# Siverteh/semantic-slam-master

Measured on AMD Instinct MI355X. Metric: frames/sec extract+match on TUM 640x480; match-index bit-exact vs CPU ref, higher is better.
Workload: dtype f32

## Files before the change

### include/sslam_hip.h

```cpp
#ifndef SSLAM_HIP_H
#define SSLAM_HIP_H

#include <stdint.h>

#ifdef __cplusplus
extern "C" {
#endif

#define SSLAM_OK 0
#define SSLAM_E_INVALID (-1)
#define SSLAM_E_UNSUPPORTED (-2)
#define SSLAM_E_LAUNCH (-3)

#define SSLAM_C 384
#define SSLAM_HID 384
#define SSLAM_D 128

int sslam_version(void);
const char *sslam_arch(void);
long long sslam_launch_count(void);

long long sslam_workspace_bytes(int n_frames, int G, int K, int n_pairs);
long long sslam_selector_saliency_workspace_bytes(int n_frames, int G);
long long sslam_sim_argmax_workspace_bytes(int n2, int n_pairs);

int sslam_test_set_knob(const char *name, long long value, int unset);

int sslam_pack_conv3x3_host(const float *w_host, int hs, float *out_host);
int sslam_pack_linear_host(const float *w_host, int n_out, int k_in, float *out_host);

#define SSLAM_MAX_TAPS 32
int sslam_resample_table_host(int in_size, int out_size, int filter, int32_t *bounds_host, int32_t *coefs_host,
                              int coefs_capacity);
int sslam_preprocess_u8(const uint8_t *img, int n, int h, int w, int size, const int32_t *bounds_h,
                        const int32_t *coefs_h, int ksize_h, const int32_t *bounds_v, const int32_t *coefs_v,
                        int ksize_v, float *out_chw, void *stream);
int sslam_preprocess_u8_patches(const uint8_t *img, int n, int h, int w, int size, const int32_t *bounds_h,
                                const int32_t *coefs_h, int ksize_h, const int32_t *bounds_v, const int32_t *coefs_v,
                                int ksize_v, void *out_patches_bf16, void *stream);

int sslam_bn_tokens(const float *tokens, int n_frames, int tokens_per_frame, int n_prefix, int group,
                    const float *gamma, const float *beta, const float *run_mean, const float *run_var, int train,
                    float eps, float *out_feat, float *out_mean, float *out_var, void *stream);

int sslam_selector_saliency(const float *feat, int n_frames, int G, const float *w1_packed, const float *b1,
                            const float *w2, const float *b2, int hs, float *sal, void *stream);
int sslam_selector_saliency_ws(const float *feat, int n_frames, int G, const float *w1_packed, const float *b1,
                               const float *w2, const float *b2, int hs, float *sal, void *workspace,
                               long long workspace_bytes, void *stream);

int sslam_f32_to_bf16(const float *in, void *out_bf16, long long n, void *stream);
int sslam_bn_tokens_bf16copy(const float *tokens, int n_frames, int tokens_per_frame, int n_prefix, int group,
                             const float *gamma, const float *beta, const float *run_mean, const float *run_var, int train,
                             float eps, float *out_feat, void *out_feat_bf16, float *out_mean, float *out_var, void *stream);
int sslam_pack_conv3x3_bf16_host(const float *w_host, int hs, void *out_bf16_host);
int sslam_selector_saliency_bf16(const void *feat_bf16, int n_frames, int G, const void *w1_packed_bf16, const float *b1,
                                 const float *w2, const float *b2, int hs, float *sal, void *stream);

int sslam_select_keypoints(const float *sal, int n_frames, int G, int K, int nms_radius, double min_score_percentile,
                           float *kp_xy, float *scores, int32_t *idx, float *kp_pixel, int32_t *status,
                           void *stream);

int sslam_gather(const float *feat, int n_frames, int G, const float *kp_xy, int K, float *out, void *stream);

typedef struct {
    int n_blocks;
    long long total;
    long long in_w, in_b;
    long long blk[8][8];
    long long out_w, out_b;
} sslam_refiner_layout_t;
int sslam_refiner_layout(int n_blocks, sslam_refiner_layout_t *layout_host);
int sslam_refiner_pack_host(const float *const *w_host, int n_blocks, float *out_host);
int sslam_refine(const float *x, long long rows, const float *packed, int n_blocks, float *desc, void *stream);

int sslam_gather_refine(const float *feat, int n_frames, int G, const float *kp_xy, int K, const float *packed,
                        int n_blocks, float *desc, void *stream);

long long sslam_refiner_bf16_bytes(int n_blocks);
int sslam_refiner_pack_bf16_host(const float *const *w_host, int n_blocks, void *out_host);
int sslam_refine_bf16(const float *x, long long rows, const void *packed_bf16, int n_blocks, float *desc, void *stream);
int sslam_gather_refine_bf16(const float *feat, int n_frames, int G, const float *kp_xy, int K, const void *packed_bf16,
                             int n_blocks, float *desc, void *stream);

int sslam_keypoint_intensity(const uint8_t *img, int n, int h, int w, int size, const int32_t *bounds_h,
                             const int32_t *coefs_h, int ksize_h, const int32_t *bounds_v, const int32_t *coefs_v,
                             int ksize_v, const float *kp_pixel, int K, float *out, void *stream);

int sslam_sim_argmax(const float *desc1, long long stride1, int n1, const float *desc2, long long stride2, int n2,
                     int n_pairs, int32_t *nn12, float *s12, int32_t *nn21, float *s21, float *second12, void *stream);
int sslam_sim_argmax_ws(const float *desc1, long long stride1, int n1, const float *desc2, long long stride2, int n2,
                        int n_pairs, int32_t *nn12, float *s12, int32_t *nn21, float *s21, float *second12,
                        void *workspace, long long workspace_bytes, void *stream);

int sslam_match_finalize(const int32_t *nn12, const float *s12, const int32_t *nn21, int n1, int n2, int n_pairs,
                         const float *scores1, long long sstride1, const float *scores2, long long sstride2,
                         const float *intensity1, const float *intensity2, float w_desc, float w_sal,
                         float min_saliency, float min_sim, float min_intensity, int64_t *matches, float *quality,
                         int32_t *count, void *stream);

typedef struct {
    const float *ln1_g, *ln1_b;
    const void *wqkv;
    const float *bqkv;
    const void *wo;
    const float *bo, *ln2_g, *ln2_b;
    const void *wup;
    const float *bup;
    const void *wdown;
    const float *bdown;
// ... 49 lines not shown
```

### semantic-slam-master_amd/csrc/common.h

```cpp
#pragma once

#include <hip/hip_runtime.h>
#include <stdint.h>

#include "../../include/sslam_hip.h"

typedef float f32x16 __attribute__((ext_vector_type(16)));
typedef float f32x4 __attribute__((ext_vector_type(4)));

extern long long g_sslam_launches;
static inline void sslam_count_launches(long long n) { __atomic_fetch_add(&g_sslam_launches, n, __ATOMIC_RELAXED); }

enum sslam_knob_id {
    KNOB_M1_VARIANT,
    KNOB_CONV_VARIANT,
    KNOB_CONV_LATENCY_ROWS,
    KNOB_CONV_LAT2_ROWS,
    KNOB_CONV_NO_HALO,
    KNOB_CONV_TAIL,
    KNOB_CONVBF_NO_HALO,
    KNOB_CONVBF_TAIL,
    KNOB_CONVBF_VARIANT,
    KNOB_VIT_NO_FUSED_MLP,
    KNOB_BN_FORM,
    KNOB_VIT_F32_NO_KEY_SPLIT,
    KNOB_RT_STOP,
    KNOB_COUNT
};
#define SSLAM_KNOB_UNSET (-0x7fffffffffffffffLL - 1)
extern long long g_sslam_knob[KNOB_COUNT];
static inline long long sslam_knob(int id, long long dflt) { const long long v = g_sslam_knob[id]; return v == SSLAM_KNOB_UNSET ? dflt : v; }
static inline bool sslam_knob_set(int id) { return g_sslam_knob[id] != SSLAM_KNOB_UNSET; }

#define SSLAM_CHECK_LAUNCH()                                   \
    do {                                                       \
        sslam_count_launches(1);                               \
        if (hipGetLastError() != hipSuccess) return SSLAM_E_LAUNCH; \
    } while (0)

__host__ __device__ inline int kp8(int k) { return (k & ~7) | ((k & 1) << 2) | ((k & 7) >> 1); }

__device__ __forceinline__ f32x16 mfma32(float a, float b, f32x16 c) {
    return __builtin_amdgcn_mfma_f32_32x32x2f32(a, b, c, 0, 0, 0);
}

__device__ __forceinline__ int crow(int r, int h) { return (r & 3) + 8 * (r >> 2) + 4 * h; }

__device__ __forceinline__ float bfly32(float v) {
    v = v + __shfl_xor(v, 16);
    v = v + __shfl_xor(v, 8);
    v = v + __shfl_xor(v, 4);
    v = v + __shfl_xor(v, 2);
    v = v + __shfl_xor(v, 1);
    return v;
}
__device__ __forceinline__ float bfly64(float v) {
    v = v + __shfl_xor(v, 32);
    return bfly32(v);
}
// ... 24 lines not shown
```

### semantic-slam-master_amd/csrc/lib.hip

```cpp
#include <stdlib.h>
#include <string.h>

#include "common.h"

long long g_sslam_launches = 0;
long long g_sslam_knob[KNOB_COUNT];

namespace {
long long g_knob_at_load[KNOB_COUNT];
const char *const kKnobNames[KNOB_COUNT] = {
    "SSLAM_M1_VARIANT",   "SSLAM_CONV_VARIANT",  "SSLAM_CONV_LATENCY_ROWS", "SSLAM_CONV_LAT2_ROWS",   "SSLAM_CONV_NO_HALO",
    "SSLAM_CONV_TAIL",    "SSLAM_CONVBF_NO_HALO", "SSLAM_CONVBF_TAIL",      "SSLAM_CONVBF_VARIANT",   "SSLAM_VIT_NO_FUSED_MLP",
    "SSLAM_BN_FORM",      "SSLAM_VIT_F32_NO_KEY_SPLIT", "SSLAM_RT_STOP"};
struct KnobInit {
    KnobInit() {
        for (int i = 0; i < KNOB_COUNT; i++) {
            const char *e = getenv(kKnobNames[i]);
            g_sslam_knob[i] = g_knob_at_load[i] = e ? atoll(e) : SSLAM_KNOB_UNSET;
        }
    }
} g_knob_init;
}

extern "C" int sslam_version(void) { return 300; }
extern "C" const char *sslam_arch(void) { return "gfx950"; }
extern "C" long long sslam_launch_count(void) { return __atomic_load_n(&g_sslam_launches, __ATOMIC_RELAXED); }

extern "C" long long sslam_workspace_bytes(int n_frames, int G, int K, int n_pairs) {
    if (n_frames <= 0 || G <= 0 || K <= 0 || n_pairs < 0) return SSLAM_E_INVALID;
    const long long a = sslam_selector_saliency_workspace_bytes(n_frames, G);
    const long long b = n_pairs > 0 ? sslam_sim_argmax_workspace_bytes(K, n_pairs) : 0;
    const long long m = a > b ? a : b;
    return (m + 255) & ~255LL;
}

extern "C" int sslam_test_set_knob(const char *name, long long value, int unset) {
    if (!name) return SSLAM_E_INVALID;
    for (int i = 0; i < KNOB_COUNT; i++)
        if (!strcmp(name, kKnobNames[i])) {
            g_sslam_knob[i] = unset ? g_knob_at_load[i] : value;
            return SSLAM_OK;
        }
    return SSLAM_E_INVALID;
}
```

### semantic-slam-master_amd/csrc/refine.hip

```cpp
#include "common.h"
#include "gather_taps.h"

namespace {

#ifndef SSLAM_REFINE_WMR
#define SSLAM_REFINE_WMR 1
#endif
constexpr int WMR = SSLAM_REFINE_WMR;
constexpr int RM = 32 * WMR;
constexpr int NTHR = 256 * WMR;
constexpr int HID = SSLAM_HID;
constexpr int LDH = HID + 4;
constexpr int NKG = HID / 8;
constexpr int H_FLOATS = RM * LDH;
constexpr int SCRATCH_FLOATS = 256;
constexpr int SMEM_FLOATS = H_FLOATS + SCRATCH_FLOATS;

struct RefArgs {
    const float *packed;
    sslam_refiner_layout_t lay;
};

typedef unsigned u32x4 __attribute__((ext_vector_type(4)));

// ... 28 lines not shown
    f32x4 an = *reinterpret_cast<const f32x4 *>(A);
#pragma unroll 1
    for (int g = 0; g < NKG; g += 3) {
        LOAD_B(b2, g + 2);
        __builtin_amdgcn_sched_barrier(0);
        STEP(b0, g);
        __builtin_amdgcn_sched_barrier(0);
        LOAD_B(b0, min(g + 3, NKG - 1));
        __builtin_amdgcn_sched_barrier(0);
        STEP(b1, g + 1);
        __builtin_amdgcn_sched_barrier(0);
        LOAD_B(b1, min(g + 4, NKG - 1));
        __builtin_amdgcn_sched_barrier(0);
        STEP(b2, g + 2);
        __builtin_amdgcn_sched_barrier(0);
    }
#undef LOAD_B
#undef STEP
}

template <int V>
struct IC {
    static constexpr int value = V;
};
template <int DW>
__device__ __forceinline__ void store_quad(unsigned row_lds, float y0, float y1, float y2, float y3) {
    asm volatile("ds_write2_b32 %0, %1, %2 offset0:%3 offset1:%4" ::"v"(row_lds), "v"(y0), "v"(y1), "n"(DW), "n"(DW + 4) : "memory");
    asm volatile("ds_write2_b32 %0, %1, %2 offset0:%3 offset1:%4" ::"v"(row_lds), "v"(y2), "v"(y3), "n"(DW + 1), "n"(DW + 5) : "memory");
}
__device__ __forceinline__ void lds_quads_done() { asm volatile("s_waitcnt lgkmcnt(0)" ::: "memory"); }
__device__ __forceinline__ unsigned lds_addr(const float *p) {
    return (unsigned)(size_t)(__attribute__((address_space(3))) const float *)p;
}
template <int I>
__device__ __forceinline__ void store_rows_from(unsigned row_lds, const f32x16 (&v)[3]) {
    if constexpr (I < 12) {
        constexpr int t = I / 4, q = I % 4;
        store_quad<32 * t + 8 * q>(row_lds, v[t][4 * q], v[t][4 * q + 1], v[t][4 * q + 2], v[t][4 * q + 3]);
        store_rows_from<I + 1>(row_lds, v);
    }
}
__device__ __forceinline__ void store_rows(float *H, int tid, const f32x16 (&v)[3]) {
    const int lane = tid & 63, wave = tid >> 6, r = lane & 31, h = lane >> 5, wn = wave & 3;
    store_rows_from<0>(lds_addr(H + r * LDH + wn * 96 + 2 * h), v);
    lds_quads_done();
}

__device__ __forceinline__ float row_total(float p, float *part, int tid) {
    const int lane = tid & 63, wave = tid >> 6, r = lane & 31, h = lane >> 5, wn = wave & 3;
    p = p + __shfl_xor(p, 32);
    if (h == 0) part[wn * 32 + r] = p;
    __syncthreads();
    return ((part[r] + part[32 + r]) + part[64 + r]) + part[96 + r];
}

__device__ __forceinline__ void layernorm_store(float *H, float *part0, float *part1, const float *__restrict__ gam,
                                                const float *__restrict__ bet, int tid, const f32x16 (&v)[3]) {
    const int lane = tid & 63, wave = tid >> 6, r = lane & 31, h = lane >> 5, wn = wave & 3;
    const float *gp = gam + wn * 96 + 4 * h, *bp = bet + wn * 96 + 4 * h;
    constexpr int AHEAD = 3;
    f32x4 g4[AHEAD], b4[AHEAD];
#define LN_REQ(i_)                                                                                       \
    {                                                                                                    \
        g4[(i_) % AHEAD] = *reinterpret_cast<const f32x4 *>(gp + 32 * ((i_) / 4) + 8 * ((i_) % 4));      \
        b4[(i_) % AHEAD] = *reinterpret_cast<const f32x4 *>(bp + 32 * ((i_) / 4) + 8 * ((i_) % 4));      \
    }
// ... 20 lines not shown
        constexpr int i = decltype(ic)::value, t = i / 4, qd = i % 4;
        const f32x4 gq = g4[i % AHEAD], bq = b4[i % AHEAD];
        float y[4];
#pragma unroll
        for (int j = 0; j < 4; j++) y[j] = __builtin_fmaf((v[t][4 * qd + j] - mean) * rstd, gq[j], bq[j]);
        if constexpr (i + AHEAD < 12) LN_REQ(i + AHEAD)
        __builtin_amdgcn_sched_barrier(0);
        store_quad<32 * t + 8 * qd>(row_lds, y[0], y[1], y[2], y[3]);
    };
    quad(IC<0>{}); quad(IC<1>{}); quad(IC<2>{}); quad(IC<3>{}); quad(IC<4>{}); quad(IC<5>{});
    quad(IC<6>{}); quad(IC<7>{}); quad(IC<8>{}); quad(IC<9>{}); quad(IC<10>{}); quad(IC<11>{});
    lds_quads_done();
#undef LN_REQ
}

#ifdef SSLAM_CLOCK_PROBE
__device__ unsigned long long g_probe_refine[8 * 4096];
#define PROBE_BEGIN() const unsigned long long pr_t0 = clock64(); unsigned long long pr_q = 0, pr_acc[6] = {0, 0, 0, 0, 0, 0}
#define PROBE(slot, stmt) { pr_q = clock64(); stmt; pr_acc[slot] += clock64() - pr_q; }
#define PROBE_END()                                                                                         \
    if (threadIdx.x == 0 && blockIdx.x < 4096) {                                                            \
        g_probe_refine[8 * blockIdx.x] = clock64() - pr_t0;                                                 \
        for (int i_ = 0; i_ < 6; i_++) g_probe_refine[8 * blockIdx.x + 1 + i_] = pr_acc[i_];                \
    }
#else
#define PROBE_BEGIN()
#define PROBE(slot, stmt) { stmt; }
#define PROBE_END()
#endif
#define PRIO_OTHER() __builtin_amdgcn_s_setprio(1)
#define PRIO_GEMM() __builtin_amdgcn_s_setprio(0)
enum { PR_GATHER = 0, PR_GEMM = 1, PR_LN = 2, PR_STORE = 3, PR_BARRIER = 4 };

__global__ __launch_bounds__(NTHR, WMR == 1 ? 3 : 2) void gather_refine_kernel(const float *__restrict__ feat, int G,
                                                             const float *__restrict__ kp_xy, int K,
                                                             const float *__restrict__ x_in, long long rows,
                                                             RefArgs args, float *__restrict__ desc) {
    __shared__ __attribute__((aligned(16))) float smem[SMEM_FLOATS];
    float *H = smem, *scratch = smem + H_FLOATS;
    const int tid = threadIdx.x;
    PROBE_BEGIN();
    PRIO_OTHER();
    long long R0;
    {
        const int n_tiles = gridDim.x, b = blockIdx.x, q = n_tiles / 8, rem = n_tiles % 8, x = b % 8;
        R0 = (long long)((x < rem ? x * (q + 1) : rem * (q + 1) + (x - rem) * q) + b / 8) * RM;
    }
    const float *pk = args.packed;
    const sslam_refiner_layout_t &L = args.lay;
    const __amdgpu_buffer_rsrc_t wrs = __builtin_amdgcn_make_buffer_rsrc(const_cast<float *>(pk), 0, (int)(L.total * 4), 0x00020000);

    {
        const int row = tid >> 3, part = tid & 7;
        long long R = R0 + row;
        if (R > rows - 1) R = rows - 1;
        float *dst = H + row * LDH;
        if (feat) {
            const long long f = R / K;
            const Taps t = make_taps(feat + f * G * G * SSLAM_C, G, kp_xy[2 * R], kp_xy[2 * R + 1]);
#pragma unroll
            for (int j = 0; j < 6; j++) {
                const int c0 = 8 * (j * 8 + part);
                float4 ev, od;
                kp8_split(blend4(t, c0), blend4(t, c0 + 4), ev, od);
                *reinterpret_cast<float4 *>(dst + c0) = ev;
                *reinterpret_cast<float4 *>(dst + c0 + 4) = od;
            }
        } else {
            const float *src = x_in + R * SSLAM_C;
#pragma unroll
            for (int j = 0; j < 6; j++) {
                const int c0 = 8 * (j * 8 + part);
                float4 ev, od;
                kp8_split(*reinterpret_cast<const float4 *>(src + c0), *reinterpret_cast<const float4 *>(src + c0 + 4), ev, od);
                *reinterpret_cast<float4 *>(dst + c0) = ev;
                *reinterpret_cast<float4 *>(dst + c0 + 4) = od;
            }
        }
    }
#ifdef SSLAM_CLOCK_PROBE
    pr_acc[PR_GATHER] = clock64() - pr_t0;
#endif
    PROBE(PR_BARRIER, __syncthreads();)

    float *part0 = scratch, *part1 = scratch + 128;
    f32x16 X[3], acc[3];
    PRIO_GEMM(); PROBE(PR_GEMM, gemm_lds<3>(H, wrs, (int)L.in_w * 4, pk + L.in_b, tid, acc);) PRIO_OTHER();
#pragma unroll
    for (int t = 0; t < 3; t++)
#pragma unroll
        for (int e = 0; e < 16; e++) X[t][e] = acc[t][e] > 0.0f ? acc[t][e] : 0.0f;

    for (int b = 0; b < L.n_blocks; b++) {
        PROBE(PR_LN, layernorm_store(H, part0, part1, pk + L.blk[b][0], pk + L.blk[b][1], tid, X);)
        PROBE(PR_BARRIER, __syncthreads();)
        PRIO_GEMM(); PROBE(PR_GEMM, gemm_lds<3>(H, wrs, (int)L.blk[b][2] * 4, pk + L.blk[b][3], tid, acc);) PRIO_OTHER();
#pragma unroll
        for (int t = 0; t < 3; t++)
#pragma unroll
            for (int e = 0; e < 16; e++) acc[t][e] = acc[t][e] > 0.0f ? acc[t][e] : 0.0f;
        PROBE(PR_LN, layernorm_store(H, part0, part1, pk + L.blk[b][4], pk + L.blk[b][5], tid, acc);)
        PROBE(PR_BARRIER, __syncthreads();)
        PRIO_GEMM(); PROBE(PR_GEMM, gemm_lds<3>(H, wrs, (int)L.blk[b][6] * 4, pk + L.blk[b][7], tid, acc);) PRIO_OTHER();
#pragma unroll
        for (int t = 0; t < 3; t++)
#pragma unroll
            for (int e = 0; e < 16; e++) {
                const float v = acc[t][e] + X[t][e];
                X[t][e] = v > 0.0f ? v : 0.0f;
            }
    }
    PROBE(PR_BARRIER, __syncthreads();)
    PROBE(PR_STORE, store_rows(H, tid, X);)
    PROBE(PR_BARRIER, __syncthreads();)

    f32x16 o[1];
    PRIO_GEMM(); PROBE(PR_GEMM, gemm_lds<1>(H, wrs, (int)L.out_w * 4, pk + L.out_b, tid, o);) PRIO_OTHER();
    {
        const int lane = tid & 63, wave = tid >> 6, r = lane & 31, h = lane >> 5, wn = wave & 3;
        float ss = 0.0f;
#pragma unroll
        for (int e = 0; e < 16; e++) ss = __builtin_fmaf(o[0][e], o[0][e], ss);
        const float den = fmaxf(sqrtf(row_total(ss, part0, tid)), 1e-12f);
        if (R0 + r < rows) {
#pragma unroll
            for (int q = 0; q < 4; q++) {
                f32x4 w4;
#pragma unroll
                for (int i = 0; i < 4; i++) w4[i] = o[0][4 * q + i] / den;
                *reinterpret_cast<f32x4 *>(desc + (R0 + r) * SSLAM_D + wn * 32 + 8 * q + 4 * h) = w4;
            }
        }
    }
    PROBE_END();
}

__global__ __launch_bounds__(256) void gather_kernel(const float *__restrict__ feat, int G, const float *__restrict__ kp_xy,
                                                      int K, long long rows, float *__restrict__ out) {
    const long long item = (long long)blockIdx.x * 256 + threadIdx.x;
    const long long R = item / (SSLAM_C / 4);
    if (R >= rows) return;
    const int c0 = (int)(item % (SSLAM_C / 4)) * 4;
    const long long f = R / K;
    const Taps t = make_taps(feat + f * G * G * SSLAM_C, G, kp_xy[2 * R], kp_xy[2 * R + 1]);
    *reinterpret_cast<float4 *>(out + R * SSLAM_C + c0) = blend4(t, c0);
}

int launch_refine(const float *feat, int G, const float *kp_xy, int K, const float *x_in, long long rows,
                  const float *packed, int n_blocks, float *desc, void *stream) {
    RefArgs a;
    a.packed = packed;
    if (sslam_refiner_layout(n_blocks, &a.lay) != SSLAM_OK) return SSLAM_E_UNSUPPORTED;
    const unsigned grid = (unsigned)((rows + RM - 1) / RM);
    hipLaunchKernelGGL(gather_refine_kernel, dim3(grid), dim3(NTHR), 0, (hipStream_t)stream, feat, G, kp_xy, K, x_in, rows,
                       a, desc);
    SSLAM_CHECK_LAUNCH();
    return SSLAM_OK;
}

}

extern "C" int sslam_refiner_layout(int n_blocks, sslam_refiner_layout_t *L) {
    if (!L || n_blocks < 0 || n_blocks > 8) return SSLAM_E_INVALID;
    long long off = 0;
    auto take = [&](long long n) { const long long o = off; off += n; return o; };
    L->n_blocks = n_blocks;
    L->in_w = take((long long)HID * SSLAM_C);
    L->in_b = take(HID);
    for (int b = 0; b < 8; b++)
        for (int k = 0; k < 8; k++) L->blk[b][k] = 0;
    for (int b = 0; b < n_blocks; b++) {
        L->blk[b][0] = take(HID); L->blk[b][1] = take(HID);
        L->blk[b][2] = take((long long)HID * HID); L->blk[b][3] = take(HID);
        L->blk[b][4] = take(HID); L->blk[b][5] = take(HID);
        L->blk[b][6] = take((long long)HID * HID); L->blk[b][7] = take(HID);
    }
    L->out_w = take((long long)SSLAM_D * HID);
    L->out_b = take(SSLAM_D);
    L->total = off;
    return SSLAM_OK;
}

extern "C" int sslam_pack_linear_host(const float *w, int n_out, int k_in, float *out) {
    if (!w || !out || n_out <= 0 || k_in <= 0 || (k_in % 8)) return SSLAM_E_INVALID;
    for (int n = 0; n < n_out; n++)
        for (int k = 0; k < k_in; k++)
            out[((long long)(k / 8) * n_out + n) * 8 + kp8(k % 8)] = w[(long long)n * k_in + k];
    return SSLAM_OK;
// ... 1 lines not shown

extern "C" int sslam_refiner_pack_host(const float *const *w, int n_blocks, float *out) {
    sslam_refiner_layout_t L;
    if (!w || !out || sslam_refiner_layout(n_blocks, &L) != SSLAM_OK) return SSLAM_E_INVALID;
    auto cp = [&](long long off, const float *src, int n) { for (int i = 0; i < n; i++) out[off + i] = src[i]; };
    sslam_pack_linear_host(w[0], HID, SSLAM_C, out + L.in_w);
    cp(L.in_b, w[1], HID);
    for (int b = 0; b < n_blocks; b++) {
        const float *const *p = w + 2 + 8 * b;
        cp(L.blk[b][0], p[0], HID); cp(L.blk[b][1], p[1], HID);
        sslam_pack_linear_host(p[2], HID, HID, out + L.blk[b][2]); cp(L.blk[b][3], p[3], HID);
        cp(L.blk[b][4], p[4], HID); cp(L.blk[b][5], p[5], HID);
        sslam_pack_linear_host(p[6], HID, HID, out + L.blk[b][6]); cp(L.blk[b][7], p[7], HID);
    }
    const float *const *po = w + 2 + 8 * n_blocks;
    sslam_pack_linear_host(po[0], SSLAM_D, HID, out + L.out_w);
    cp(L.out_b, po[1], SSLAM_D);
    return SSLAM_OK;
}

extern "C" int sslam_refine(const float *x, long long rows, const float *packed, int n_blocks, float *desc, void *stream) {
    if (!x || !packed || !desc || rows <= 0) return SSLAM_E_INVALID;
    if (((uintptr_t)x | (uintptr_t)packed) & 15) return SSLAM_E_INVALID;
    return launch_refine(nullptr, 0, nullptr, 1, x, rows, packed, n_blocks, desc, stream);
}

extern "C" int sslam_gather_refine(const float *feat, int n_frames, int G, const float *kp_xy, int K, const float *packed,
                                   int n_blocks, float *desc, void *stream) {
    if (!feat || !kp_xy || !packed || !desc || n_frames <= 0 || G <= 1 || K <= 0) return SSLAM_E_INVALID;
    if (((uintptr_t)feat | (uintptr_t)packed) & 15) return SSLAM_E_INVALID;
    return launch_refine(feat, G, kp_xy, K, nullptr, (long long)n_frames * K, packed, n_blocks, desc, stream);
}

extern "C" int sslam_gather(const float *feat, int n_frames, int G, const float *kp_xy, int K, float *out, void *stream) {
    if (!feat || !kp_xy || !out || n_frames <= 0 || G <= 1 || K <= 0) return SSLAM_E_INVALID;
    if (((uintptr_t)feat | (uintptr_t)out) & 15) return SSLAM_E_INVALID;
    const long long rows = (long long)n_frames * K, items = rows * (SSLAM_C / 4);
    hipLaunchKernelGGL(gather_kernel, dim3((unsigned)((items + 255) / 256)), dim3(256), 0, (hipStream_t)stream, feat, G, kp_xy,
                       K, rows, out);
    SSLAM_CHECK_LAUNCH();
    return SSLAM_OK;
}

#ifdef SSLAM_CLOCK_PROBE
extern "C" int sslam_probe_refine(unsigned long long *host) {
    return hipMemcpyFromSymbol(host, HIP_SYMBOL(g_probe_refine), sizeof(unsigned long long) * 8 * 4096) == hipSuccess ? 0 : -3;
}
#endif
```

### semantic-slam-master_amd/sslam_amd/lib.py

```python
from __future__ import annotations

import ctypes as C
import os
import subprocess

import numpy as np
import torch

_PKG = os.path.dirname(os.path.dirname(os.path.abspath(__file__)))
CSRC = os.path.join(_PKG, "csrc")
SO_PATH = os.path.join(CSRC, "libsslam_hip.so")

OK, E_INVALID, E_UNSUPPORTED, E_LAUNCH = 0, -1, -2, -3
_ERR = {E_INVALID: "invalid argument", E_UNSUPPORTED: "unsupported shape", E_LAUNCH: "kernel launch failed"}

C_FEAT, HID, D_OUT = 384, 384, 128
MAX_TAPS = 32


class SslamHipError(RuntimeError):
    pass


class VitLayer(C.Structure):
# ... 12 lines not shown


class VitWeightsF32(C.Structure):
    _fields_ = [("patch_w", C.c_void_p), ("patch_b", C.c_void_p), ("prefix", C.c_void_p), ("layer", VitLayerF32 * 12),
                ("norm_g", C.c_void_p), ("norm_b", C.c_void_p), ("rope_cos", C.c_void_p), ("rope_sin", C.c_void_p)]


class RefinerLayout(C.Structure):
    _fields_ = [("n_blocks", C.c_int), ("total", C.c_longlong), ("in_w", C.c_longlong), ("in_b", C.c_longlong),
                ("blk", (C.c_longlong * 8) * 8), ("out_w", C.c_longlong), ("out_b", C.c_longlong)]


def build(force: bool = False) -> str:
    srcs = [os.path.join(CSRC, f) for f in os.listdir(CSRC) if f.endswith((".hip", ".h"))]
    srcs.append(os.path.join(os.path.dirname(_PKG), "include", "sslam_hip.h"))
    stale = (not os.path.exists(SO_PATH)) or any(os.path.getmtime(s) > os.path.getmtime(SO_PATH) for s in srcs)
    if force or stale:
        subprocess.check_call(["make", "-C", CSRC, "-s", "-j4"])
    return SO_PATH


_lib = None

EXPORTS = [
    "sslam_version", "sslam_arch", "sslam_launch_count", "sslam_pack_conv3x3_host", "sslam_pack_linear_host",
    "sslam_resample_table_host", "sslam_preprocess_u8", "sslam_bn_tokens", "sslam_selector_saliency",
    "sslam_select_keypoints", "sslam_gather", "sslam_refiner_layout", "sslam_refiner_pack_host", "sslam_refine",
    "sslam_gather_refine", "sslam_keypoint_intensity", "sslam_sim_argmax", "sslam_match_finalize",
    "sslam_vit_pack_linear_host", "sslam_vit_pack_mlp_host", "sslam_vit_workspace_bytes", "sslam_vit_forward",
    "sslam_f32_to_bf16", "sslam_pack_conv3x3_bf16_host", "sslam_selector_saliency_bf16",
    "sslam_bn_tokens_bf16copy", "sslam_refiner_bf16_bytes", "sslam_refiner_pack_bf16_host", "sslam_refine_bf16", "sslam_gather_refine_bf16",
    "sslam_workspace_bytes", "sslam_selector_saliency_workspace_bytes", "sslam_sim_argmax_workspace_bytes",
    "sslam_selector_saliency_ws", "sslam_sim_argmax_ws", "sslam_test_set_knob",
    "sslam_preprocess_u8_patches", "sslam_vit_forward_patches", "sslam_vit_f32_workspace_bytes", "sslam_vit_forward_f32",
    "sslam_vit_f32_pack_linear_host", "sslam_vit_forward_f32_form",
    "sslam_vit_workspace_bytes_form", "sslam_vit_forward_form", "sslam_vit_forward_patches_form",
]


def lib():
    global _lib
    if _lib is None:
        if not os.path.exists(SO_PATH):
            raise SslamHipError(f"{SO_PATH} is missing: run `python -c 'import __graft_entry__ as g; g.build()'` "
                                f"(or `make -C {CSRC}`); this package has no non-HIP execution path")
        L = C.CDLL(SO_PATH)
        L.sslam_arch.restype = C.c_char_p
        L.sslam_launch_count.restype = C.c_longlong
        p, i, ll, f, d = C.c_void_p, C.c_int, C.c_longlong, C.c_float, C.c_double
        L.sslam_pack_conv3x3_host.argtypes = [p, i, p]
        L.sslam_pack_linear_host.argtypes = [p, i, i, p]
        L.sslam_resample_table_host.argtypes = [i, i, i, p, p, i]
        L.sslam_preprocess_u8.argtypes = [p, i, i, i, i, p, p, i, p, p, i, p, p]
        L.sslam_preprocess_u8_patches.argtypes = [p, i, i, i, i, p, p, i, p, p, i, p, p]
        L.sslam_bn_tokens.argtypes = [p, i, i, i, i, p, p, p, p, i, f, p, p, p, p]
        L.sslam_selector_saliency.argtypes = [p, i, i, p, p, p, p, i, p, p]
        L.sslam_selector_saliency_ws.argtypes = [p, i, i, p, p, p, p, i, p, p, ll, p]
        for fn, at in ((L.sslam_workspace_bytes, [i, i, i, i]), (L.sslam_selector_saliency_workspace_bytes, [i, i]),
                       (L.sslam_sim_argmax_workspace_bytes, [i, i])):
            fn.restype, fn.argtypes = ll, at
        L.sslam_test_set_knob.argtypes = [C.c_char_p, ll, i]
        L.sslam_select_keypoints.argtypes = [p, i, i, i, i, d, p, p, p, p, p, p]
        L.sslam_gather.argtypes = [p, i, i, p, i, p, p]
        L.sslam_refiner_layout.argtypes = [i, C.POINTER(RefinerLayout)]
        L.sslam_refiner_pack_host.argtypes = [p, i, p]
        L.sslam_refine.argtypes = [p, ll, p, i, p, p]
        L.sslam_gather_refine.argtypes = [p, i, i, p, i, p, i, p, p]
        L.sslam_keypoint_intensity.argtypes = [p, i, i, i, i, p, p, i, p, p, i, p, i, p, p]
        L.sslam_sim_argmax.argtypes = [p, ll, i, p, ll, i, i, p, p, p, p, p, p]
        L.sslam_sim_argmax_ws.argtypes = [p, ll, i, p, ll, i, i, p, p, p, p, p, p, ll, p]
        L.sslam_match_finalize.argtypes = [p, p, p, i, i, i, p, ll, p, ll, p, p, f, f, f, f, f, p, p, p, p]
        L.sslam_f32_to_bf16.argtypes = [p, p, ll, p]
        L.sslam_pack_conv3x3_bf16_host.argtypes = [p, i, p]
        L.sslam_selector_saliency_bf16.argtypes = [p, i, i, p, p, p, p, i, p, p]
        L.sslam_bn_tokens_bf16copy.argtypes = [p, i, i, i, i, p, p, p, p, i, f, p, p, p, p, p]
        L.sslam_refiner_bf16_bytes.restype = C.c_longlong
        L.sslam_refiner_bf16_bytes.argtypes = [i]
        L.sslam_refiner_pack_bf16_host.argtypes = [p, i, p]
        L.sslam_refine_bf16.argtypes = [p, ll, p, i, p, p]
        L.sslam_gather_refine_bf16.argtypes = [p, i, i, p, i, p, i, p, p]
        L.sslam_vit_pack_linear_host.argtypes = [p, i, i, p]
        L.sslam_vit_pack_mlp_host.argtypes = [p, p, p, p]
        L.sslam_vit_workspace_bytes.restype = C.c_longlong
        L.sslam_vit_workspace_bytes.argtypes = [i, i]
        L.sslam_vit_forward.argtypes = [p, i, i, C.POINTER(VitWeights), p, ll, p, p]
        L.sslam_vit_forward_patches.argtypes = [p, i, i, C.POINTER(VitWeights), p, ll, p, p]
        L.sslam_vit_workspace_bytes_form.restype = C.c_longlong
        L.sslam_vit_workspace_bytes_form.argtypes = [i, i, i]
        L.sslam_vit_forward_form.argtypes = [p, i, i, C.POINTER(VitWeights), p, ll, p, i, p]
        L.sslam_vit_forward_patches_form.argtypes = [p, i, i, C.POINTER(VitWeights), p, ll, p, i, p]
        L.sslam_vit_f32_workspace_bytes.restype = C.c_longlong
        L.sslam_vit_f32_workspace_bytes.argtypes = [i, i]
        L.sslam_vit_forward_f32.argtypes = [p, i, i, C.POINTER(VitWeightsF32), p, ll, p, p]
        L.sslam_vit_forward_f32_form.argtypes = [p, i, i, C.POINTER(VitWeightsF32), p, ll, p, i, p]
        L.sslam_vit_f32_pack_linear_host.argtypes = [p, i, i, p]
        _lib = L
    return _lib


def _check(rc: int, what: str):
# ... 208 lines not shown
    if out is not None:
        kp, sc, idx, px, st = out
    else:
        kp = torch.empty((n, K, 2), dtype=torch.float32, device=dev)
        sc = torch.empty((n, K), dtype=torch.float32, device=dev)
        idx = torch.empty((n, K), dtype=torch.int32, device=dev) if want_idx else None
        px = torch.empty((n, K, 2), dtype=torch.float32, device=dev) if want_pixel else None
        st = torch.empty((n,), dtype=torch.int32, device=dev)
    _run("select_keypoints", lib().sslam_select_keypoints, (sal, kp, sc, idx, px, st,),
         _dp(sal), n, g, K, radius, C.c_double(pct), _dp(kp), _dp(sc), _dp(idx), _dp(px),
                                        _dp(st))
    return kp, sc, idx, px, st


def gather(feat, kp, out=None):
    n, g = feat.shape[0], feat.shape[1]
    K = kp.shape[1]
    if out is None:
        out = torch.empty((n, K, C_FEAT), dtype=torch.float32, device=feat.device)
    _run("gather", lib().sslam_gather, (feat, kp, out,),
         _dp(feat), n, g, _dp(kp), K, _dp(out))
    return out


def refine(x, packed, n_blocks, out=None):
    rows = x.numel() // C_FEAT
    if out is None:
        out = torch.empty(x.shape[:-1] + (D_OUT,), dtype=torch.float32, device=x.device)
    _run("refine", lib().sslam_refine, (x, packed, out,),
         _dp(x), rows, _dp(packed), n_blocks, _dp(out))
    return out


def gather_refine(feat, kp, packed, n_blocks, out=None):
    n, g = feat.shape[0], feat.shape[1]
    K = kp.shape[1]
    if out is None:
        out = torch.empty((n, K, D_OUT), dtype=torch.float32, device=feat.device)
    _run("gather_refine", lib().sslam_gather_refine, (feat, kp, packed, out,),
         _dp(feat), n, g, _dp(kp), K, _dp(packed), n_blocks, _dp(out))
    return out


def gather_refine_bf16(feat, kp, packed_bf16, n_blocks, out=None):
    n, g = feat.shape[0], feat.shape[1]
    K = kp.shape[1]
    if out is None:
        out = torch.empty((n, K, D_OUT), dtype=torch.float32, device=feat.device)
    _run("gather_refine_bf16", lib().sslam_gather_refine_bf16, (feat, kp, packed_bf16, out,),
         _dp(feat), n, g, _dp(kp), K, _dp(packed_bf16), n_blocks, _dp(out))
    return out


def refine_bf16(x, packed_bf16, n_blocks, out=None):
    rows = x.shape[0]
    if out is None:
        out = torch.empty((rows, D_OUT), dtype=torch.float32, device=x.device)
    _run("refine_bf16", lib().sslam_refine_bf16, (x, packed_bf16, out,),
         _dp(x), rows, _dp(packed_bf16), n_blocks, _dp(out))
    return out


def keypoint_intensity(img, size, tab_h, tab_v, kp_pixel, out=None):
    n, h, w, _ = img.shape
    K = kp_pixel.shape[1]
    if out is None:
        out = torch.empty((n, K), dtype=torch.float32, device=img.device)
    (bh, ch, kh), (bv, cv, kv) = tab_h, tab_v
    _run("keypoint_intensity", lib().sslam_keypoint_intensity, (img, bh, ch, bv, cv, kp_pixel, out,),
         _dp(img), n, h, w, size, _dp(bh), _dp(ch), kh, _dp(bv), _dp(cv), kv, _dp(kp_pixel), K,
                                          _dp(out))
    return out


# ... 120 lines not shown
```

### semantic-slam-master_amd/sslam_amd/pipeline.py

```python
from __future__ import annotations

from dataclasses import dataclass

import numpy as np
import torch

from . import lib

PATCH = 16
N_PREFIX = 5
MAX_PAIRS_PER_LAUNCH = 65535


@dataclass
class ExtractorConfig:
    input_size: int = 448
    num_keypoints: int = 500
    nms_radius: int = 2
    min_score_percentile: float = 0.50
    bn_train_mode: bool = True
    bn_eps: float = 1e-5
    saliency_weight: float = 0.3
    min_saliency: float = 0.5
    min_descriptor_sim: float = 0.7
# ... 243 lines not shown
                   status=torch.empty((n,), dtype=torch.int32, device=dev))
        if with_intensity:
            out["intensity"] = torch.empty((n, K), **f32)
        return out

    def extract(self, tokens: torch.Tensor, images_u8: torch.Tensor | None = None, out: dict | None = None,
                images_ready: "torch.cuda.Event | None" = None) -> dict:
        n, step = tokens.shape[0], self.launch_group()
        if out is None:
            out = self.alloc_extract(n, images_u8 is not None)
        for a in range(0, n, step):
            b = min(a + step, n)
            self._extract_group(tokens[a:b], None if images_u8 is None else images_u8[a:b], {k: v[a:b] for k, v in out.items()},
                                images_ready if a == 0 else None)
        if self.cfg.num_keypoints > self.cfg.grid ** 2 and bool(out["status"].any()):
            raise RuntimeError("selected index k out of range")
        return out

    def _extract_group(self, tokens: torch.Tensor, images_u8: torch.Tensor | None, out: dict, images_ready=None) -> None:
        cfg, s = self.cfg, self.selector
        ws = self.workspace(tokens.shape[0], 0)
        if self.bf16:
            feat, feat_bf = self.features(tokens, bf16_copy=True, reuse=True)
            lib.selector_saliency_bf16(feat_bf, s.w1p_bf16, s.b1, s.w2, s.b2, s.hidden, out=out["saliency"])
            del feat_bf
        else:
            feat = self.features(tokens, reuse=True)
            lib.selector_saliency(feat, s.w1p, s.b1, s.w2, s.b2, s.hidden, out=out["saliency"], workspace=ws)
        lib.select_keypoints(out["saliency"], cfg.num_keypoints, cfg.nms_radius, cfg.min_score_percentile,
                             out=(out["keypoints_patch"], out["scores"], out["idx"], out["keypoints_pixel"], out["status"]))
        if self.bf16:
            lib.gather_refine_bf16(feat, out["keypoints_patch"], self.refiner.packed_bf16, self.refiner.n_blocks, out=out["descriptors"])
        else:
            lib.gather_refine(feat, out["keypoints_patch"], self.refiner.packed, self.refiner.n_blocks, out=out["descriptors"])
        if images_ready is not None:
            torch.cuda.current_stream(self.device).wait_event(images_ready)
        if images_u8 is not None and "intensity" in out:
            n, h, w, _ = images_u8.shape
            th, tv = self.tables.get(h, w, cfg.input_size, True)
            lib.keypoint_intensity(images_u8, cfg.input_size, th, tv, out["keypoints_pixel"], out=out["intensity"])

    def alloc_match(self, n_pairs: int, k: int | None = None) -> dict:
        k = self.cfg.num_keypoints if k is None else k
        dev = self.device
        return dict(matches=torch.empty((n_pairs, k, 2), dtype=torch.int64, device=dev),
                    quality=torch.empty((n_pairs, k), dtype=torch.float32, device=dev),
                    match_count=torch.empty((n_pairs,), dtype=torch.int32, device=dev))

    def match(self, desc, scores, intensity=None, spacing: int | None = None, out: dict | None = None) -> dict:
        cfg = self.cfg
        sp = cfg.spacing if spacing is None else spacing
        n, k = desc.shape[0], desc.shape[1]
        n_pairs = n - sp
        if n_pairs <= 0:
            z = torch.zeros
            return dict(matches=z((0, k, 2), dtype=torch.int64, device=desc.device),
                        quality=z((0, k), dtype=torch.float32, device=desc.device),
                        match_count=z((0,), dtype=torch.int32, device=desc.device))
        use_int = cfg.use_intensity and intensity is not None
        res = dict(out) if out is not None else self.alloc_match(n_pairs, k)
        aux = []
        for a in range(0, n_pairs, MAX_PAIRS_PER_LAUNCH):
            m = min(MAX_PAIRS_PER_LAUNCH, n_pairs - a)
            d1, d2 = desc[a:a + m], desc[a + sp:a + sp + m]
            nn12, s12, nn21, _, _ = lib.sim_argmax(d1, k * lib.D_OUT, k, d2, k * lib.D_OUT, k, m, workspace=self.workspace(0, m))
            lib.match_finalize(nn12, s12, nn21, k, k, m, scores[a:], k, scores[a + sp:], k,
                               intensity[a:] if use_int else None, intensity[a + sp:] if use_int else None,
# ... 24 lines not shown
```

Measured before the change: 57210.

## Deduplicate identical keypoints before refiner MLP and copy descriptors to duplicates

Adds a hash-based pass that finds, per frame, keypoints with bit-identical coordinates. The refiner kernel then runs only over a compacted list of distinct rows, and a copy kernel fills in the descriptors of duplicate rows. This avoids recomputing the per-row MLP for repeated keypoints, at the cost of three extra launches and workspace. It is enabled by default only when the row count is large, and it also swaps the ReLU select for an inline v_max instruction.

Result: faster. 58430 (median of 6 runs) (+2.1%).

```diff
diff --git a/include/sslam_hip.h b/include/sslam_hip.h
--- a/include/sslam_hip.h
+++ b/include/sslam_hip.h
@@ -22,6 +22,7 @@
 
 long long sslam_workspace_bytes(int n_frames, int G, int K, int n_pairs);
 long long sslam_selector_saliency_workspace_bytes(int n_frames, int G);
+long long sslam_gather_refine_workspace_bytes(int n_frames, int K);
 long long sslam_sim_argmax_workspace_bytes(int n2, int n_pairs);
 
 int sslam_test_set_knob(const char *name, long long value, int unset);
@@ -76,6 +77,8 @@
 
 int sslam_gather_refine(const float *feat, int n_frames, int G, const float *kp_xy, int K, const float *packed,
                         int n_blocks, float *desc, void *stream);
+int sslam_gather_refine_ws(const float *feat, int n_frames, int G, const float *kp_xy, int K, const float *packed,
+                           int n_blocks, float *desc, void *workspace, long long workspace_bytes, void *stream);
 
 long long sslam_refiner_bf16_bytes(int n_blocks);
 int sslam_refiner_pack_bf16_host(const float *const *w_host, int n_blocks, void *out_host);
diff --git a/semantic-slam-master_amd/csrc/common.h b/semantic-slam-master_amd/csrc/common.h
--- a/semantic-slam-master_amd/csrc/common.h
+++ b/semantic-slam-master_amd/csrc/common.h
@@ -25,6 +25,7 @@
     KNOB_BN_FORM,
     KNOB_VIT_F32_NO_KEY_SPLIT,
     KNOB_RT_STOP,
+    KNOB_REFINE_DISTINCT,
     KNOB_COUNT
 };
 #define SSLAM_KNOB_UNSET (-0x7fffffffffffffffLL - 1)
diff --git a/semantic-slam-master_amd/csrc/lib.hip b/semantic-slam-master_amd/csrc/lib.hip
--- a/semantic-slam-master_amd/csrc/lib.hip
+++ b/semantic-slam-master_amd/csrc/lib.hip
@@ -11,7 +11,8 @@
 const char *const kKnobNames[KNOB_COUNT] = {
     "SSLAM_M1_VARIANT",   "SSLAM_CONV_VARIANT",  "SSLAM_CONV_LATENCY_ROWS", "SSLAM_CONV_LAT2_ROWS",   "SSLAM_CONV_NO_HALO",
     "SSLAM_CONV_TAIL",    "SSLAM_CONVBF_NO_HALO", "SSLAM_CONVBF_TAIL",      "SSLAM_CONVBF_VARIANT",   "SSLAM_VIT_NO_FUSED_MLP",
-    "SSLAM_BN_FORM",      "SSLAM_VIT_F32_NO_KEY_SPLIT", "SSLAM_RT_STOP"};
+    "SSLAM_BN_FORM",      "SSLAM_VIT_F32_NO_KEY_SPLIT", "SSLAM_RT_STOP",
+    "SSLAM_REFINE_DISTINCT"};
 struct KnobInit {
     KnobInit() {
         for (int i = 0; i < KNOB_COUNT; i++) {
@@ -30,7 +31,8 @@
     if (n_frames <= 0 || G <= 0 || K <= 0 || n_pairs < 0) return SSLAM_E_INVALID;
     const long long a = sslam_selector_saliency_workspace_bytes(n_frames, G);
     const long long b = n_pairs > 0 ? sslam_sim_argmax_workspace_bytes(K, n_pairs) : 0;
-    const long long m = a > b ? a : b;
+    const long long c = sslam_gather_refine_workspace_bytes(n_frames, K);
+    const long long m = a > b ? (a > c ? a : c) : (b > c ? b : c);
     return (m + 255) & ~255LL;
 }
 
diff --git a/semantic-slam-master_amd/csrc/refine.hip b/semantic-slam-master_amd/csrc/refine.hip
--- a/semantic-slam-master_amd/csrc/refine.hip
+++ b/semantic-slam-master_amd/csrc/refine.hip
@@ -84,6 +84,11 @@
 __device__ __forceinline__ unsigned lds_addr(const float *p) {
     return (unsigned)(size_t)(__attribute__((address_space(3))) const float *)p;
 }
+__device__ __forceinline__ float relu(float x) {
+    float y;
+    asm("v_max_f32 %0, 0, %1" : "=v"(y) : "v"(x));
+    return y;
+}
 template <int I>
 __device__ __forceinline__ void store_rows_from(unsigned row_lds, const f32x16 (&v)[3]) {
     if constexpr (I < 12) {
@@ -170,18 +175,26 @@
 #define PRIO_GEMM() __builtin_amdgcn_s_setprio(0)
 enum { PR_GATHER = 0, PR_GEMM = 1, PR_LN = 2, PR_STORE = 3, PR_BARRIER = 4 };
 
+template <bool WL>
 __global__ __launch_bounds__(NTHR, WMR == 1 ? 3 : 2) void gather_refine_kernel(const float *__restrict__ feat, int G,
                                                              const float *__restrict__ kp_xy, int K,
                                                              const float *__restrict__ x_in, long long rows,
+                                                             const int *__restrict__ list, const int *__restrict__ n_list,
                                                              RefArgs args, float *__restrict__ desc) {
     __shared__ __attribute__((aligned(16))) float smem[SMEM_FLOATS];
     float *H = smem, *scratch = smem + H_FLOATS;
     const int tid = threadIdx.x;
+    int n_tiles = gridDim.x;
+    if constexpr (WL) {
+        rows = *n_list;
+        n_tiles = (int)((rows + RM - 1) / RM);
+        if ((int)blockIdx.x >= n_tiles) return;
+    }
     PROBE_BEGIN();
     PRIO_OTHER();
     long long R0;
     {
-        const int n_tiles = gridDim.x, b = blockIdx.x, q = n_tiles / 8, rem = n_tiles % 8, x = b % 8;
+        const int b = blockIdx.x, q = n_tiles / 8, rem = n_tiles % 8, x = b % 8;
         R0 = (long long)((x < rem ? x * (q + 1) : rem * (q + 1) + (x - rem) * q) + b / 8) * RM;
     }
     const float *pk = args.packed;
@@ -192,6 +205,7 @@
         const int row = tid >> 3, part = tid & 7;
         long long R = R0 + row;
         if (R > rows - 1) R = rows - 1;
+        if constexpr (WL) R = list[R];
         float *dst = H + row * LDH;
         if (feat) {
             const long long f = R / K;
@@ -227,7 +241,7 @@
 #pragma unroll
     for (int t = 0; t < 3; t++)
 #pragma unroll
-        for (int e = 0; e < 16; e++) X[t][e] = acc[t][e] > 0.0f ? acc[t][e] : 0.0f;
+        for (int e = 0; e < 16; e++) X[t][e] = relu(acc[t][e]);
 
     for (int b = 0; b < L.n_blocks; b++) {
         PROBE(PR_LN, layernorm_store(H, part0, part1, pk + L.blk[b][0], pk + L.blk[b][1], tid, X);)
@@ -236,7 +250,7 @@
 #pragma unroll
         for (int t = 0; t < 3; t++)
 #pragma unroll
-            for (int e = 0; e < 16; e++) acc[t][e] = acc[t][e] > 0.0f ? acc[t][e] : 0.0f;
+            for (int e = 0; e < 16; e++) acc[t][e] = relu(acc[t][e]);
         PROBE(PR_LN, layernorm_store(H, part0, part1, pk + L.blk[b][4], pk + L.blk[b][5], tid, acc);)
         PROBE(PR_BARRIER, __syncthreads();)
         PRIO_GEMM(); PROBE(PR_GEMM, gemm_lds<3>(H, wrs, (int)L.blk[b][6] * 4, pk + L.blk[b][7], tid, acc);) PRIO_OTHER();
@@ -261,12 +275,14 @@
         for (int e = 0; e < 16; e++) ss = __builtin_fmaf(o[0][e], o[0][e], ss);
         const float den = fmaxf(sqrtf(row_total(ss, part0, tid)), 1e-12f);
         if (R0 + r < rows) {
+            long long Ro = R0 + r;
+            if constexpr (WL) Ro = list[Ro];
 #pragma unroll
             for (int q = 0; q < 4; q++) {
                 f32x4 w4;
 #pragma unroll
                 for (int i = 0; i < 4; i++) w4[i] = o[0][4 * q + i] / den;
-                *reinterpret_cast<f32x4 *>(desc + (R0 + r) * SSLAM_D + wn * 32 + 8 * q + 4 * h) = w4;
+                *reinterpret_cast<f32x4 *>(desc + Ro * SSLAM_D + wn * 32 + 8 * q + 4 * h) = w4;
             }
         }
     }
@@ -284,14 +300,158 @@
     *reinterpret_cast<float4 *>(out + R * SSLAM_C + c0) = blend4(t, c0);
 }
 
+constexpr int DN = 256;
+constexpr int DISTINCT_MAX_K = 4096;
+constexpr long long DISTINCT_MIN_ROWS = 256 * 3 * RM + 1;
+
+__device__ __forceinline__ bool is_nan_bits(unsigned u) { return (u & 0x7fffffffu) > 0x7f800000u; }
+__device__ __forceinline__ unsigned hash_xy(unsigned x, unsigned y) {
+    unsigned h = x * 0x9e3779b1u ^ (y + 0x7f4a7c15u) * 0x85ebca6bu;
+    h ^= h >> 15;
+    h *= 0x2c1b3c6du;
+    return h ^ (h >> 13);
+}
+__device__ __forceinline__ int block_sum(int v, int *red, int tid) {
+#pragma unroll
+    for (int o = 32; o >= 1; o >>= 1) v += __shfl_xor(v, o);
+    __syncthreads();
+    if ((tid & 63) == 0) red[tid >> 6] = v;
+    __syncthreads();
+    int s = 0;
+#pragma unroll
+    for (int w = 0; w < DN / 64; w++) s += red[w];
+    return s;
+}
+
+__global__ __launch_bounds__(DN) void distinct_rep_kernel(const unsigned *__restrict__ kp_bits, int K, int T,
+                                                          int *__restrict__ rep, int *__restrict__ counts) {
+    extern __shared__ int tab[];
+    __shared__ int red[DN / 64];
+    const int tid = threadIdx.x, f = blockIdx.x, mask = T - 1;
+    const unsigned *kp = kp_bits + 2ll * f * K;
+    for (int i = tid; i < T; i += DN) tab[i] = -1;
+    __syncthreads();
+    for (int j = tid; j < K; j += DN) {
+        const unsigned x = kp[2 * j], y = kp[2 * j + 1];
+        if (is_nan_bits(x) || is_nan_bits(y)) continue;
+        for (unsigned h = hash_xy(x, y) & mask;; h = (h + 1) & mask) {
+            const int cur = atomicCAS(&tab[h], -1, j);
+            if (cur == -1) break;
+            if (kp[2 * cur] == x && kp[2 * cur + 1] == y) {
+                atomicMin(&tab[h], j);
+                break;
+            }
+        }
+    }
+    __syncthreads();
+    int n = 0;
+    for (int j = tid; j < K; j += DN) {
+        const unsigned x = kp[2 * j], y = kp[2 * j + 1];
+        int r = j;
+        if (!(is_nan_bits(x) || is_nan_bits(y)))
+            for (unsigned h = hash_xy(x, y) & mask;; h = (h + 1) & mask) {
+                const int cur = tab[h];
+                if (cur < 0) break;
+                if (kp[2 * cur] == x && kp[2 * cur + 1] == y) {
+                    r = cur;
+                    break;
+                }
+            }
+        rep[(long long)f * K + j] = f * K + r;
+        n += r == j;
+    }
+    n = block_sum(n, red, tid);
+    if (tid == 0) counts[f] = n;
+}
+
+__global__ __launch_bounds__(DN) void distinct_list_kernel(const int *__restrict__ rep, int K, int n_frames,
+                                                           int *__restrict__ counts, int *__restrict__ list) {
+    __shared__ int red[DN / 64];
+    const int tid = threadIdx.x, f = blockIdx.x, lane = tid & 63;
+    int before = 0;
+    for (int i = tid; i < f; i += DN) before += counts[i];
+    before = block_sum(before, red, tid);
+    const int chunk = (K + DN - 1) / DN, b = min(tid * chunk, K), e = min(b + chunk, K), R0 = f * K;
+    int local = 0;
+    for (int j = b; j < e; j++) local += rep[R0 + j] == R0 + j;
+    int incl = local;
+#pragma unroll
+    for (int o = 1; o < 64; o <<= 1) {
+        const int up = __shfl_up(incl, o);
+        if (lane >= o) incl += up;
+    }
+    __syncthreads();
+    if (lane == 63) red[tid >> 6] = incl;
+    __syncthreads();
+    int slot = before + incl - local;
+    for (int w = 0; w < (tid >> 6); w++) slot += red[w];
+    for (int j = b; j < e; j++)
+        if (rep[R0 + j] == R0 + j) list[slot++] = R0 + j;
+    if (f == n_frames - 1 && tid == DN - 1) counts[n_frames] = slot;
+}
+
+__global__ __launch_bounds__(256) void copy_duplicates_kernel(const int *__restrict__ rep, long long rows, float *desc) {
+    const long long item = (long long)blockIdx.x * 256 + threadIdx.x;
+    const long long R = item / (SSLAM_D / 4);
+    if (R >= rows) return;
+    const long long src = rep[R];
+    if (src == R) return;
+    const int c0 = (int)(item % (SSLAM_D / 4)) * 4;
+    *reinterpret_cast<float4 *>(desc + R * SSLAM_D + c0) = *reinterpret_cast<const float4 *>(desc + src * SSLAM_D + c0);
+}
+
+struct DistinctWs {
+    long long counts, rep, list, bytes;
+};
+DistinctWs distinct_ws(int n_frames, long long rows) {
+    auto up = [](long long b) { return (b + 255) & ~255LL; };
+    DistinctWs w;
+    w.counts = 0;
+    w.rep = up(((long long)n_frames + 1) * 4);
+    w.list = w.rep + up(rows * 4);
+    w.bytes = w.list + up(rows * 4);
+    return w;
+}
+bool distinct_form(int n_frames, int K) {
+    const long long rows = (long long)n_frames * K;
+    if (K > DISTINCT_MAX_K || rows > 0x7fffffffLL) return false;
+    const long long forced = sslam_knob(KNOB_REFINE_DISTINCT, -1);
+    return forced < 0 ? rows >= DISTINCT_MIN_ROWS : forced != 0;
+}
+
 int launch_refine(const float *feat, int G, const float *kp_xy, int K, const float *x_in, long long rows,
                   const float *packed, int n_blocks, float *desc, void *stream) {
     RefArgs a;
     a.packed = packed;
     if (sslam_refiner_layout(n_blocks, &a.lay) != SSLAM_OK) return SSLAM_E_UNSUPPORTED;
     const unsigned grid = (unsigned)((rows + RM - 1) / RM);
-    hipLaunchKernelGGL(gather_refine_kernel, dim3(grid), dim3(NTHR), 0, (hipStream_t)stream, feat, G, kp_xy, K, x_in, rows,
-                       a, desc);
+    hipLaunchKernelGGL(gather_refine_kernel<false>, dim3(grid), dim3(NTHR), 0, (hipStream_t)stream, feat, G, kp_xy, K, x_in,
+                       rows, (const int *)nullptr, (const int *)nullptr, a, desc);
+    SSLAM_CHECK_LAUNCH();
+    return SSLAM_OK;
+}
+
+int launch_refine_distinct(const float *feat, int n_frames, int G, const float *kp_xy, int K, const float *packed, int n_blocks,
+                           float *desc, void *workspace, void *stream) {
+    RefArgs a;
+    a.packed = packed;
+    if (sslam_refiner_layout(n_blocks, &a.lay) != SSLAM_OK) return SSLAM_E_UNSUPPORTED;
+    const long long rows = (long long)n_frames * K;
+    const DistinctWs w = distinct_ws(n_frames, rows);
+    int *counts = (int *)((char *)workspace + w.counts), *rep = (int *)((char *)workspace + w.rep),
+        *list = (int *)((char *)workspace + w.list);
+    int T = 64;
+    while (T < 2 * K) T <<= 1;
+    hipStream_t st = (hipStream_t)stream;
+    hipLaunchKernelGGL(distinct_rep_kernel, dim3(n_frames), dim3(DN), (size_t)T * 4, st, (const unsigned *)kp_xy, K, T, rep, counts);
+    SSLAM_CHECK_LAUNCH();
+    hipLaunchKernelGGL(distinct_list_kernel, dim3(n_frames), dim3(DN), 0, st, rep, K, n_frames, counts, list);
+    SSLAM_CHECK_LAUNCH();
+    const unsigned grid = (unsigned)((rows + RM - 1) / RM);
+    hipLaunchKernelGGL(gather_refine_kernel<true>, dim3(grid), dim3(NTHR), 0, st, feat, G, kp_xy, K, (const float *)nullptr, rows,
+                       (const int *)list, (const int *)(counts + n_frames), a, desc);
+    SSLAM_CHECK_LAUNCH();
+    hipLaunchKernelGGL(copy_duplicates_kernel, dim3((unsigned)((rows * (SSLAM_D / 4) + 255) / 256)), dim3(256), 0, st, rep, rows, desc);
     SSLAM_CHECK_LAUNCH();
     return SSLAM_OK;
 }
@@ -359,6 +519,21 @@
     return launch_refine(feat, G, kp_xy, K, nullptr, (long long)n_frames * K, packed, n_blocks, desc, stream);
 }
 
+extern "C" long long sslam_gather_refine_workspace_bytes(int n_frames, int K) {
+    if (n_frames <= 0 || K <= 0) return SSLAM_E_INVALID;
+    return distinct_form(n_frames, K) ? distinct_ws(n_frames, (long long)n_frames * K).bytes : 0;
+}
+
+extern "C" int sslam_gather_refine_ws(const float *feat, int n_frames, int G, const float *kp_xy, int K, const float *packed,
+                                      int n_blocks, float *desc, void *workspace, long long workspace_bytes, void *stream) {
+    if (!feat || !kp_xy || !packed || !desc || n_frames <= 0 || G <= 1 || K <= 0) return SSLAM_E_INVALID;
+    if (((uintptr_t)feat | (uintptr_t)packed) & 15) return SSLAM_E_INVALID;
+    if (distinct_form(n_frames, K) && workspace && !((uintptr_t)workspace & 3) &&
+        workspace_bytes >= distinct_ws(n_frames, (long long)n_frames * K).bytes)
+        return launch_refine_distinct(feat, n_frames, G, kp_xy, K, packed, n_blocks, desc, workspace, stream);
+    return launch_refine(feat, G, kp_xy, K, nullptr, (long long)n_frames * K, packed, n_blocks, desc, stream);
+}
+
 extern "C" int sslam_gather(const float *feat, int n_frames, int G, const float *kp_xy, int K, float *out, void *stream) {
     if (!feat || !kp_xy || !out || n_frames <= 0 || G <= 1 || K <= 0) return SSLAM_E_INVALID;
     if (((uintptr_t)feat | (uintptr_t)out) & 15) return SSLAM_E_INVALID;
diff --git a/semantic-slam-master_amd/sslam_amd/lib.py b/semantic-slam-master_amd/sslam_amd/lib.py
--- a/semantic-slam-master_amd/sslam_amd/lib.py
+++ b/semantic-slam-master_amd/sslam_amd/lib.py
@@ -68,6 +68,7 @@
     "sslam_bn_tokens_bf16copy", "sslam_refiner_bf16_bytes", "sslam_refiner_pack_bf16_host", "sslam_refine_bf16", "sslam_gather_refine_bf16",
     "sslam_workspace_bytes", "sslam_selector_saliency_workspace_bytes", "sslam_sim_argmax_workspace_bytes",
     "sslam_selector_saliency_ws", "sslam_sim_argmax_ws", "sslam_test_set_knob",
+    "sslam_gather_refine_ws", "sslam_gather_refine_workspace_bytes",
     "sslam_preprocess_u8_patches", "sslam_vit_forward_patches", "sslam_vit_f32_workspace_bytes", "sslam_vit_forward_f32",
     "sslam_vit_f32_pack_linear_host", "sslam_vit_forward_f32_form",
     "sslam_vit_workspace_bytes_form", "sslam_vit_forward_form", "sslam_vit_forward_patches_form",
@@ -93,7 +94,7 @@
         L.sslam_selector_saliency.argtypes = [p, i, i, p, p, p, p, i, p, p]
         L.sslam_selector_saliency_ws.argtypes = [p, i, i, p, p, p, p, i, p, p, ll, p]
         for fn, at in ((L.sslam_workspace_bytes, [i, i, i, i]), (L.sslam_selector_saliency_workspace_bytes, [i, i]),
-                       (L.sslam_sim_argmax_workspace_bytes, [i, i])):
+                       (L.sslam_sim_argmax_workspace_bytes, [i, i]), (L.sslam_gather_refine_workspace_bytes, [i, i])):
             fn.restype, fn.argtypes = ll, at
         L.sslam_test_set_knob.argtypes = [C.c_char_p, ll, i]
         L.sslam_select_keypoints.argtypes = [p, i, i, i, i, d, p, p, p, p, p, p]
@@ -102,6 +103,7 @@
         L.sslam_refiner_pack_host.argtypes = [p, i, p]
         L.sslam_refine.argtypes = [p, ll, p, i, p, p]
         L.sslam_gather_refine.argtypes = [p, i, i, p, i, p, i, p, p]
+        L.sslam_gather_refine_ws.argtypes = [p, i, i, p, i, p, i, p, p, ll, p]
         L.sslam_keypoint_intensity.argtypes = [p, i, i, i, i, p, p, i, p, p, i, p, i, p, p]
         L.sslam_sim_argmax.argtypes = [p, ll, i, p, ll, i, i, p, p, p, p, p, p]
         L.sslam_sim_argmax_ws.argtypes = [p, ll, i, p, ll, i, i, p, p, p, p, p, p, ll, p]
@@ -376,14 +378,20 @@
     return out
 
 
-def gather_refine(feat, kp, packed, n_blocks, out=None):
+def gather_refine(feat, kp, packed, n_blocks, out=None, workspace=None):
     n, g = feat.shape[0], feat.shape[1]
     K = kp.shape[1]
     if out is None:
         out = torch.empty((n, K, D_OUT), dtype=torch.float32, device=feat.device)
-    _run("gather_refine", lib().sslam_gather_refine, (feat, kp, packed, out,),
-         _dp(feat), n, g, _dp(kp), K, _dp(packed), n_blocks, _dp(out))
-    return out
+    ws, wsb = _scratch(workspace, int(lib().sslam_gather_refine_workspace_bytes(n, K)), feat.device)
+    _run("gather_refine", lib().sslam_gather_refine_ws, (feat, kp, packed, out, ws),
+         _dp(feat), n, g, _dp(kp), K, _dp(packed), n_blocks, _dp(out), _dp(ws), wsb)
+    return out
+
+
+def gather_refine_counts(workspace, n_frames: int):
+    c = workspace[: 4 * (n_frames + 1)].view(torch.int32)
+    return c[:n_frames], c[n_frames]
 
 
 def gather_refine_bf16(feat, kp, packed_bf16, n_blocks, out=None):
diff --git a/semantic-slam-master_amd/sslam_amd/pipeline.py b/semantic-slam-master_amd/sslam_amd/pipeline.py
--- a/semantic-slam-master_amd/sslam_amd/pipeline.py
+++ b/semantic-slam-master_amd/sslam_amd/pipeline.py
@@ -299,7 +299,7 @@
         if self.bf16:
             lib.gather_refine_bf16(feat, out["keypoints_patch"], self.refiner.packed_bf16, self.refiner.n_blocks, out=out["descriptors"])
         else:
-            lib.gather_refine(feat, out["keypoints_patch"], self.refiner.packed, self.refiner.n_blocks, out=out["descriptors"])
+            lib.gather_refine(feat, out["keypoints_patch"], self.refiner.packed, self.refiner.n_blocks, out=out["descriptors"], workspace=ws)
         if images_ready is not None:
             torch.cuda.current_stream(self.device).wait_event(images_ready)
         if images_u8 is not None and "intensity" in out:
```
